# francescofugazzi/3dgsconverter

Measured on AMD Instinct MI355X. Metric: Msplats/sec SOR k=16, higher is better.
Workload: dtype f32 select / f64 finalize

## Files before the change

3dgsconverter_amd/csrc/knn_mfma.h:

```cpp
#pragma once

#include <hip/hip_runtime.h>

namespace gsx {

__device__ __forceinline__ unsigned shift_in_lt(unsigned m, float qx, float qy, float qz, float px, float py,
                                                float pz, float neg_tau)
{
    const float dx = qx - px, dy = qy - py, dz = qz - pz;
    const float t = __builtin_fmaf(dz, dz, __builtin_fmaf(dy, dy, __builtin_fmaf(dx, dx, neg_tau)));
    return __builtin_amdgcn_alignbit(m, __float_as_uint(t), 31);
}

typedef __bf16 bf16x8 __attribute__((ext_vector_type(8)));
typedef float f32x16 __attribute__((ext_vector_type(16)));
typedef unsigned u32x4 __attribute__((ext_vector_type(4)));
constexpr float MF_SLACK = 1e-3f;

__device__ __forceinline__ unsigned cvt_pk_bf16(float lo, float hi)
{
    unsigned r;
    asm("v_cvt_pk_bf16_f32 %0, %1, %2" : "=v"(r) : "v"(lo), "v"(hi));
    return r;
}
__device__ __forceinline__ float bf_lo(unsigned w) { return __uint_as_float(w << 16); }
__device__ __forceinline__ float bf_hi(unsigned w) { return __uint_as_float(w & 0xffff0000u); }

__host__ __device__ constexpr int mf_cand_of_row(int r) { return (r & 3) | (((r >> 3) & 3) << 2) | (((r >> 2) & 1) << 4); }

__device__ __forceinline__ bf16x8 mf_candidate_operand(float ux, float uy, float uz, bool upper)
{
    const unsigned l0 = cvt_pk_bf16(ux, ux);
    const float lx = ux - bf_lo(l0);
    const unsigned l1 = cvt_pk_bf16(lx, uy);
    const float ly = uy - bf_hi(l1);
    const unsigned l2 = cvt_pk_bf16(uy, ly);
    const unsigned l3 = cvt_pk_bf16(uz, uz);
    const float lz = uz - bf_lo(l3);
    const float n = __builtin_fmaf(uz, uz, __builtin_fmaf(uy, uy, ux * ux));
    const unsigned u0 = cvt_pk_bf16(lz, n);
    const float r1 = n - bf_hi(u0);
    const unsigned t = cvt_pk_bf16(r1, r1);
    const float r2 = r1 - bf_lo(t);
    const unsigned u1 = cvt_pk_bf16(r1, r2);
    u32x4 w;
    w.x = upper ? u0 : l0;
    w.y = upper ? u1 : l1;
    w.z = upper ? 0x3f803f80u : l2;
    w.w = upper ? 0x00003f80u : l3;
    return __builtin_bit_cast(bf16x8, w);
}

__device__ __forceinline__ void mf_query_operands(float ux, float uy, float uz, float s, bf16x8 &out_a, bf16x8 &out_b)
{
    const unsigned hx = cvt_pk_bf16(ux, uy);
    const unsigned hz = cvt_pk_bf16(uz, uz);
    const float hxf = bf_lo(hx), hyf = bf_hi(hx), hzf = bf_lo(hz);
    const float lx = ux - hxf, ly = uy - hyf, lz = uz - hzf;
    u32x4 lo, up;
    lo.x = cvt_pk_bf16(-2.0f * hxf, -2.0f * lx);
    lo.y = cvt_pk_bf16(-2.0f * hxf, -2.0f * hyf);
    lo.z = cvt_pk_bf16(-2.0f * ly, -2.0f * hyf);
    lo.w = cvt_pk_bf16(-2.0f * hzf, -2.0f * lz);
    const unsigned t1 = cvt_pk_bf16(s, s);
    const float r1 = s - bf_lo(t1);
    const unsigned t2 = cvt_pk_bf16(r1, r1);
    const float r2 = r1 - bf_lo(t2);
    up.x = cvt_pk_bf16(-2.0f * hzf, 1.0f);
    up.y = 0x3f803f80u;
    up.z = cvt_pk_bf16(s, r1);
    up.w = cvt_pk_bf16(r2, 0.0f);
    u32x4 a, b;
#pragma unroll
    for (int i = 0; i < 4; ++i) {
        auto r = __builtin_amdgcn_permlane32_swap(lo[i], up[i], false, false);
        a[i] = r[0];
        b[i] = r[1];
    }
    out_a = __builtin_bit_cast(bf16x8, a);
    out_b = __builtin_bit_cast(bf16x8, b);
}

__device__ __forceinline__ unsigned mf_sign_bits(const f32x16 &acc)
{
    unsigned m = 0;
#pragma unroll
    for (int r = 0; r < 16; ++r) m = __builtin_amdgcn_alignbit(m, __float_as_uint(acc[r]), 31);
    return m;
}

__device__ __forceinline__ void wave_sync()
{
    __builtin_amdgcn_fence(__ATOMIC_ACQ_REL, "wavefront");
    __builtin_amdgcn_wave_barrier();
}

}
```

3dgsconverter_amd/csrc/sor_grid.hip:

```cpp
#include <algorithm>
#include <chrono>
#include <cmath>
#include <cstdlib>
#include <type_traits>
#include <unordered_map>
#include <vector>

#include "gsx_common.h"
#include "knn_common.h"
#include "knn_mfma.h"
#include "sor_grid_params.h"

namespace gsx {


constexpr int MAX_DIM = 1024;
constexpr int MAX_BUCKETS = 4096;
constexpr int MAX_BUCKET_CELLS = 4096;
#ifndef GSX_BUCKET_POINTS
#define GSX_BUCKET_POINTS 4096
#endif
constexpr int BUCKET_POINTS = GSX_BUCKET_POINTS;
#ifndef GSX_BIN_TILE
#define GSX_BIN_TILE 8192
// ... 556 lines not shown
}

#ifndef GSX_SORT_THREADS
#define GSX_SORT_THREADS 512
#endif
#ifndef GSX_SORT_PPT
#define GSX_SORT_PPT 16
#endif
constexpr int SORT_THREADS = GSX_SORT_THREADS;
constexpr int SORT_PPT = GSX_SORT_PPT;
constexpr unsigned SORT_CAP = SORT_THREADS * SORT_PPT;

__device__ __forceinline__ int quarter_coord(float v, float o, float inv_h, int dim)
{
    int c = (int)((v - o) * (4.0f * inv_h));
    return min(max(c, 0), 4 * dim - 1);
}

template <bool FINE>
__global__ __launch_bounds__(SORT_THREADS) void bucket_sort_kernel(const GridParams *__restrict__ gp,
                                                          const unsigned *__restrict__ bk_start,
                                                          const float4 *__restrict__ in, float4 *__restrict__ out,
                                                          unsigned *__restrict__ cell_start, unsigned big_limit,
                                                          unsigned *__restrict__ fine_start)
{
    constexpr int SUB = FINE ? 4 : 1;
    __shared__ unsigned cnt[SUB * MAX_BUCKET_CELLS];
    __shared__ unsigned wsum[SORT_THREADS / 64];
    const GridParams g = *gp;
    const int b = blockIdx.x;
    if (g.bad_input || b >= g.bk_count) return;
    const int ncell = g.bk_cells;
    const int cells = SUB * ncell;
    const unsigned s0 = bk_start[b], s1 = bk_start[b + 1];
    if (b == g.bk_count - 1 && threadIdx.x == 0) {
        cell_start[(size_t)g.bk_count * ncell] = s1;
        if (FINE) fine_start[(size_t)g.bk_count * cells] = s1;
    }
    if (s1 - s0 > big_limit) return;
    const int by = b % g.bk_ny, bz = b / g.bk_ny;
    for (int i = threadIdx.x; i < cells; i += SORT_THREADS) cnt[i] = 0;
    __syncthreads();
    auto local_cell = [&](const float4 p) {
        const int cx = FINE ? quarter_coord(p.x, g.ox, g.inv_h, g.nx) : cell_coord(p.x, g.ox, g.inv_h, g.nx);
        const int cy = cell_coord(p.y, g.oy, g.inv_h, g.ny);
        const int cz = cell_coord(p.z, g.oz, g.inv_h, g.nz);
        return ((cz - bz * g.bk_g) * g.bk_g + (cy - by * g.bk_g)) * (SUB * g.nx) + cx;
    };
    const bool fits = s1 - s0 <= SORT_CAP;
    float4 p[SORT_PPT];
    int cell[SORT_PPT];
    unsigned rk[SORT_PPT];
    if (fits) {
#pragma unroll
        for (int u = 0; u < SORT_PPT; ++u) p[u] = in[min(s0 + u * SORT_THREADS + threadIdx.x, s1 - 1)];
#pragma unroll
        for (int u = 0; u < SORT_PPT; ++u) {
            cell[u] = local_cell(p[u]);
            rk[u] = s0 + u * SORT_THREADS + threadIdx.x < s1 ? atomicAdd(&cnt[cell[u]], 1u) : 0u;
        }
    } else {
        for (unsigned i = s0 + threadIdx.x; i < s1; i += SORT_THREADS) atomicAdd(&cnt[local_cell(in[i])], 1u);
    }
    __syncthreads();
    const int seg = (cells + SORT_THREADS - 1) / SORT_THREADS;
    const int c0 = min(cells, (int)threadIdx.x * seg), c1 = min(cells, c0 + seg);
    unsigned sum = 0;
    for (int c = c0; c < c1; ++c) sum += cnt[c];
    unsigned inc = sum;
#pragma unroll
    for (int off = 1; off < 64; off <<= 1) {
        unsigned o = __shfl_up(inc, off);
        if ((int)(threadIdx.x & 63) >= off) inc += o;
    }
    const int wv = threadIdx.x >> 6;
    if ((threadIdx.x & 63) == 63) wsum[wv] = inc;
    __syncthreads();
    unsigned run = inc - sum;
    for (int i = 0; i < wv; ++i) run += wsum[i];
    __syncthreads();
    for (int c = c0; c < c1; ++c) {
        const unsigned v = cnt[c];
        cnt[c] = run;
        run += v;
    }
    __syncthreads();
    unsigned *cs = cell_start + (size_t)b * ncell;
    for (int i = threadIdx.x; i < ncell; i += SORT_THREADS) cs[i] = s0 + cnt[SUB * i];
    if (FINE) {
        unsigned *fs = fine_start + (size_t)b * cells;
        for (int i = threadIdx.x; i < cells; i += SORT_THREADS) fs[i] = s0 + cnt[i];
    }
    if (fits) {
#pragma unroll
        for (int u = 0; u < SORT_PPT; ++u)
            if (s0 + u * SORT_THREADS + threadIdx.x < s1) out[s0 + cnt[cell[u]] + rk[u]] = p[u];
    } else {
        __syncthreads();
        for (unsigned i = s0 + threadIdx.x; i < s1; i += SORT_THREADS) {
            const float4 q = in[i];
            out[s0 + atomicAdd(&cnt[local_cell(q)], 1u)] = q;
        }
    }
}

constexpr unsigned BIG_BUCKET = 32768;
constexpr int BIG_CHUNK = 8192;

__device__ __forceinline__ int bucket_containing(const unsigned *bk_start, int nb, unsigned pos)
{
    int lo = 0, hi = nb;
    while (hi - lo > 1) {
        const int mid = (lo + hi) >> 1;
        if (bk_start[mid] <= pos) lo = mid; else hi = mid;
    }
    return lo;
}

template <bool SCATTER>
__global__ __launch_bounds__(256) void big_bucket_kernel(const GridParams *__restrict__ gp, const unsigned *__restrict__ bk_start,
                                                         int n, const float4 *__restrict__ in, float4 *__restrict__ out,
                                                         unsigned *cell_start ,
                                                         unsigned *cursor )
{
    __shared__ unsigned cnt[MAX_BUCKET_CELLS];
    __shared__ unsigned base[SCATTER ? MAX_BUCKET_CELLS : 1];
    const GridParams g = *gp;
    if (g.bad_input) return;
    const unsigned lo = (unsigned)blockIdx.x * BIG_CHUNK;
    if (lo >= (unsigned)n) return;
    const unsigned hi = min((unsigned)n, lo + BIG_CHUNK);
    const int cells = g.bk_cells;
    for (int b = bucket_containing(bk_start, g.bk_count, lo); b < g.bk_count; ++b) {
        const unsigned s0 = bk_start[b], s1 = bk_start[b + 1];
        if (s0 >= hi) break;
        if (s1 - s0 <= BIG_BUCKET) continue;
        const unsigned p0 = max(lo, s0), p1 = min(hi, s1);
        const int by = b % g.bk_ny, bz = b / g.bk_ny;
        auto local_cell = [&](const float4 p) {
            const int cx = cell_coord(p.x, g.ox, g.inv_h, g.nx);
            const int cy = cell_coord(p.y, g.oy, g.inv_h, g.ny);
            const int cz = cell_coord(p.z, g.oz, g.inv_h, g.nz);
            return ((cz - bz * g.bk_g) * g.bk_g + (cy - by * g.bk_g)) * g.nx + cx;
        };
        for (int i = threadIdx.x; i < cells; i += 256) cnt[i] = 0;
        __syncthreads();
        for (unsigned i = p0 + threadIdx.x; i < p1; i += 256) atomicAdd(&cnt[local_cell(in[i])], 1u);
        __syncthreads();
        unsigned *gc = (SCATTER ? cursor : cell_start) + (size_t)b * cells;
        for (int i = threadIdx.x; i < cells; i += 256) {
            const unsigned c = cnt[i];
            if (c) {
                const unsigned r = atomicAdd(&gc[i], c);
                if (SCATTER) base[i] = r;
            }
            if (SCATTER) cnt[i] = 0;
        }
        __syncthreads();
        if (SCATTER) {
            for (unsigned i = p0 + threadIdx.x; i < p1; i += 256) {
                const float4 p = in[i];
                const int c = local_cell(p);
                out[base[c] + atomicAdd(&cnt[c], 1u)] = p;
            }
            __syncthreads();
        }
    }
}

__global__ __launch_bounds__(256) void big_bucket_scan_kernel(const GridParams *__restrict__ gp,
                                                              const unsigned *__restrict__ bk_start,
                                                              unsigned *cell_start, unsigned *cursor)
{
    __shared__ unsigned wsum[4];
    const GridParams g = *gp;
    const int b = blockIdx.x;
    if (g.bad_input || b >= g.bk_count) return;
    const unsigned s0 = bk_start[b], s1 = bk_start[b + 1];
    if (s1 - s0 <= BIG_BUCKET) return;
    const int cells = g.bk_cells;
    unsigned *cs = cell_start + (size_t)b * cells, *cu = cursor + (size_t)b * cells;
    const int seg = (cells + 255) / 256;
    const int c0 = min(cells, (int)threadIdx.x * seg), c1 = min(cells, c0 + seg);
    unsigned sum = 0;
    for (int c = c0; c < c1; ++c) sum += cs[c];
    unsigned tot;
    unsigned run = s0 + block_exclusive_scan_256(sum, &tot, wsum);
    for (int c = c0; c < c1; ++c) {
        const unsigned v = cs[c];
        cs[c] = run;
        cu[c] = run;
        run += v;
    }
}

constexpr int PLAN_MAXQ = 64;
constexpr int PLAN_MAXRUN = 10;
constexpr int PLAN_WAVES = 4;

template <bool WRITE>
__global__ __launch_bounds__(64 * PLAN_WAVES) void brick_plan_kernel(GridParams *__restrict__ gp, const unsigned *__restrict__ fine_start,
                                                                     unsigned *__restrict__ bundle_cnt, unsigned *__restrict__ bundle_off,
                                                                     uint2 *__restrict__ list)
{
    __shared__ unsigned s_sum[PLAN_WAVES][MAX_DIM + 1];
    __shared__ unsigned short s_nxt[PLAN_WAVES][MAX_DIM];
    __shared__ unsigned wsum[4];
    __shared__ unsigned s_last;
    const GridParams g = *gp;
    if (g.bad_input || !g.plan) return;
    const int lane = threadIdx.x & 63, wv = threadIdx.x >> 6;
    unsigned *S = s_sum[wv];
    unsigned short *nxt = s_nxt[wv];
    const int nq4 = 4 * g.nx, nbund = g.nby * g.nbz;
    const unsigned cap = (unsigned)g.plan_cap;
    constexpr int QPL = MAX_DIM / 64 + 1;
    for (int bundle = (int)blockIdx.x * PLAN_WAVES + wv; bundle < nbund; bundle += (int)gridDim.x * PLAN_WAVES) {
        const int bz = bundle / g.nby, by = bundle - bz * g.nby;
        int rb[4];
#pragma unroll
        for (int r = 0; r < 4; ++r) {
            const int yy = 2 * by + (r & 1), zz = 2 * bz + (r >> 1);
            rb[r] = yy < g.ny && zz < g.nz ? 4 * row_base(g, yy, zz) : -1;
        }
        unsigned v[QPL][4];
#pragma unroll
        for (int u = 0; u < QPL; ++u) {
            const int q = lane + 64 * u;
#pragma unroll
            for (int r = 0; r < 4; ++r) v[u][r] = (q <= nq4 && rb[r] >= 0) ? fine_start[rb[r] + q] : 0u;
        }
#pragma unroll
        for (int u = 0; u < QPL; ++u) {
            const int q = lane + 64 * u;
            if (q <= nq4) S[q] = v[u][0] + v[u][1] + v[u][2] + v[u][3];
        }
        wave_sync();
        for (int s = lane; s < nq4; s += 64) {
            const unsigned s0 = S[s];
            int e = s + 1;
#pragma unroll
            for (int j = 2; j <= PLAN_MAXRUN; ++j) e += (s + j <= nq4 && S[min(s + j, nq4)] - s0 <= (unsigned)PLAN_MAXQ) ? 1 : 0;
            nxt[s] = (unsigned short)e;
        }
        wave_sync();
        if (lane == 0) {
            const unsigned base = WRITE ? bundle_off[bundle] : 0u;
            unsigned n = 0;
            for (int s = 0; s < nq4; ++n) {
                const int e = nxt[s];
                if (WRITE && base + n < cap) list[base + n] = make_uint2((unsigned)bundle, (unsigned)s | ((unsigned)(e - 1) << 16));
                s = e;
            }
            if (!WRITE) __hip_atomic_store(&bundle_cnt[bundle], n, __ATOMIC_RELAXED, __HIP_MEMORY_SCOPE_AGENT);
        }
        wave_sync();
    }
    if (WRITE) return;
    __builtin_amdgcn_s_waitcnt(0);
    __syncthreads();
    if (threadIdx.x == 0) s_last = atomicAdd(&gp->ticket_plan, 1u) == gridDim.x - 1 ? 1u : 0u;
    __syncthreads();
    if (!s_last) return;
    constexpr int HOLD = 16;
    const int seg = (nbund + 255) / 256;
    const int c0 = min(nbund, (int)threadIdx.x * seg), c1 = min(nbund, c0 + seg);
    const bool held = seg <= HOLD;
    unsigned hv[HOLD];
    unsigned sum = 0;
    for (int c = c0; c < c1; c += HOLD) {
#pragma unroll
        for (int u = 0; u < HOLD; ++u) hv[u] = c + u < c1 ? __hip_atomic_load(&bundle_cnt[c + u], __ATOMIC_RELAXED, __HIP_MEMORY_SCOPE_AGENT) : 0u;
#pragma unroll
        for (int u = 0; u < HOLD; ++u) sum += hv[u];
    }
    unsigned tot;
    unsigned run = block_exclusive_scan_256(sum, &tot, wsum);
    for (int c = c0; c < c1; c += HOLD) {
        unsigned w[HOLD];
#pragma unroll
        for (int u = 0; u < HOLD; ++u)
            w[u] = held ? hv[u] : (c + u < c1 ? __hip_atomic_load(&bundle_cnt[c + u], __ATOMIC_RELAXED, __HIP_MEMORY_SCOPE_AGENT) : 0u);
#pragma unroll
        for (int u = 0; u < HOLD; ++u) {
            if (c + u < c1) bundle_off[c + u] = run;
            run += w[u];
        }
    }
    if (threadIdx.x == 0) {
        gp->ticket_plan = 0;
        if (tot > cap) {
            gp->plan = 0;
        } else {
            gp->nbricks = (int)tot;
            gp->part_lo = 0;
            gp->part_hi = (int)tot;
        }
    }
}

#ifndef GSX_NET_WAVES17
#define GSX_NET_WAVES17 5
#endif
#ifndef GSX_BRICK_UNROLL3
#define GSX_BRICK_UNROLL3 0
#endif
#ifndef GSX_NET_WAVES33
#define GSX_NET_WAVES33 4
#endif
#ifndef GSX_NET_HB
#define GSX_NET_HB 4
#endif
#ifndef GSX_NET_WAVES25
#define GSX_NET_WAVES25 4
#endif
#ifndef GSX_NET_WAVES49
#define GSX_NET_WAVES49 3
#endif
constexpr int NET_WAVES9 = 5, NET_WAVES17 = GSX_NET_WAVES17, NET_WAVES25 = GSX_NET_WAVES25, NET_WAVES33 = GSX_NET_WAVES33,
              NET_WAVES49 = GSX_NET_WAVES49;
constexpr int NET_HB = GSX_NET_HB;
constexpr int brick_min_waves(int kcap, bool mf, bool net)
{
    (void)mf;
    if (net) return kcap <= 9 ? NET_WAVES9 : (kcap <= 17 ? NET_WAVES17 : (kcap <= 25 ? NET_WAVES25 : (kcap <= 33 ? NET_WAVES33 : (kcap <= 49 ? NET_WAVES49 : 2))));
    return kcap <= 17 ? 5 : (kcap <= 26 ? 4 : (kcap <= 33 ? 3 : 2));
}

template <int KCAP, bool EXTRA, bool MF, bool NET, bool PLAN = false>
__global__ __launch_bounds__(BRICK_THREADS, brick_min_waves(KCAP, MF, NET)) void knn_brick_kernel(
    GridParams *__restrict__ gp, const float4 *__restrict__ refs, const unsigned *__restrict__ rstart,
    const float4 *__restrict__ qpts, const unsigned *__restrict__ qstart, int k, int q_begin,
    float *__restrict__ mean_out, unsigned *__restrict__ faillist, uint2 *__restrict__ extra,
    unsigned *__restrict__ deferred, double *__restrict__ kth_out, const uint2 *__restrict__ plist)
{
    constexpr int WCAP = KCAP > 33 ? GSX_WCAP_BIG : (KCAP > 17 ? GSX_WCAP_MID : gsx::WCAP);
    __shared__ unsigned s_mask[BRICK_THREADS / 64][WCAP][64];
    __shared__ unsigned s_wbase[BRICK_THREADS / 64][WCAP];
    __shared__ uint2 s_wseg[MF ? BRICK_THREADS / 64 : 1][MF ? WCAP : 1];

    if (EXTRA && gp->extra_count == 0) return;
    const int lane = lane_id();
    const int wv = uniform((int)(threadIdx.x >> 6));
    unsigned(*mask)[64] = s_mask[wv];
    unsigned *wbase = s_wbase[wv];
    uint2 *wseg = s_wseg[MF ? wv : 0];

    const int nx = gp->nx, ny = gp->ny, nz = gp->nz;
    const int nbx = gp->nbx, nby = gp->nby;
    const int bdx = gp->bdx, bdy = gp->bdy, bdz = gp->bdz;
    const int cry = bdy + 2;
    const int ncrows = cry * (bdz + 2);
    const int nqrows = bdy * bdz;
    const double r1sq = gp->r1sq;
    const double hp = gp->hprime;
    const float tau1 = gp->tau1;
    const float g_ox = gp->ox, g_oy = gp->oy, g_oz = gp->oz, g_inv_h = gp->inv_h;
    const int bk_g = gp->bk_g, bk_ny = gp->bk_ny, bk_cells = gp->bk_cells;
    auto row_base_g = [&](int cy, int cz) {
        const int by_ = cy / bk_g, bz_ = cz / bk_g;
        return (bz_ * bk_ny + by_) * bk_cells + ((cz - bz_ * bk_g) * bk_g + (cy - by_ * bk_g)) * nx;
    };
#ifdef GSX_ABLATE
    const int dbg = gp->debug_skip;
#else
    constexpr int dbg = 0;
#endif
    const int kk = k + 1;
    const int kq = NET ? k : kk;

    WorkQueue wq;
    const int part_lo = gp->part_lo;
    const int nq4 = 4 * nx;
    const bool planned = PLAN && gp->plan != 0;
    const int dw = EXTRA ? 0 : gp->defer_words;
    wq_init(wq, EXTRA ? gp->extra_ctr : gp->brick_ctr, EXTRA ? (int)gp->extra_count : gp->part_hi - part_lo,
            BRICK_THREADS / 64);
    for (;;) {
        const int item = uniform(wq_next(wq));
        if (item < 0) break;
        int b = item + part_lo, qb = 0;
        if (EXTRA) {
            const uint2 it = extra[item];
            b = uniform((int)it.x);
            qb = uniform((int)it.y);
        }
        int bx, by, bz;
        int qf = 0, ql = 0;
        if constexpr (PLAN) {
            int bundle;
            if (planned) {
                const uint2 e = plist[b];
                bundle = uniform((int)e.x);
                qf = uniform((int)(e.y & 0xffffu));
                ql = uniform((int)(e.y >> 16));
            } else {
                bundle = b / nbx;
                qf = 8 * (b - bundle * nbx);
                ql = min(qf + 7, nq4 - 1);
            }
            bz = bundle / nby;
            by = bundle - bz * nby;
            bx = 0;
        } else {
            bz = b / (nbx * nby);
            const int brem = b - bz * nbx * nby;
            by = brem / nbx;
            bx = brem - by * nbx;
        }

        int v_start = 0, v_len = 0;
        {
            const int ln = pinned_here(lane);
            const bool isq = ln >= 16;
            const int r = isq ? ln - 16 : ln;
            const int r_mod_bdy = bdy == 2 ? (r & 1) : 0, r_div_bdy = bdy == 2 ? (r >> 1) : r;
            const int r_div_cry = cry == 4 ? (r >> 2) : (r * 11) >> 5;
            const int r_mod_cry = r - r_div_cry * cry;
            const int yy = isq ? by * bdy + r_mod_bdy : by * bdy - 1 + r_mod_cry;
            const int zz = isq ? bz * bdz + r_div_bdy : bz * bdz - 1 + r_div_cry;
            const int xa = PLAN ? (isq ? qf : max(qf - 4, 0)) : (isq ? bx * bdx : max(bx * bdx - 1, 0));
            const int xb = PLAN ? (isq ? ql : min(ql + 4, nq4 - 1))
                                : (isq ? min(bx * bdx + bdx - 1, nx - 1) : min(bx * bdx + bdx, nx - 1));
            const bool valid = (isq ? (lane < 20 && r < nqrows) : r < ncrows) && yy >= 0 && yy < ny && zz >= 0 && zz < nz;
            if (valid) {
                const unsigned *st = isq ? qstart : rstart;
                const int row = PLAN ? 4 * row_base_g(yy, zz) : row_base_g(yy, zz);
                unsigned s = st[row + xa], e = st[row + xb + 1];
                v_start = (int)s;
                v_len = (int)(e - s);
            }
        }
        if (dbg & 16) continue;
        int qoff[5];
        qoff[0] = 0;
#pragma unroll
        for (int r = 0; r < 4; ++r) qoff[r + 1] = qoff[r] + __builtin_amdgcn_readlane(v_len, 16 + r);
        const int nq = qoff[4];
        if (!EXTRA) {
            if (dw > 0 && nq > 0) {
                int ncand = 0;
#pragma unroll
                for (int r = 0; r < 16; ++r) ncand += __builtin_amdgcn_readlane(v_len, r);
                const int words = (ncand + 31) >> 5, batches = (nq + 63) >> 6;
                if (words > dw || (long long)words * batches > 2LL * dw) {
                    if (lane == 0) deferred[atomicAdd(&gp->deferred_count, 1u)] = (unsigned)b;
                    continue;
                }
            }
        }
        constexpr int LOCAL_MAX = 3;
        const int LOCAL_BATCHES = nq > 64 * LOCAL_MAX ? 1 : LOCAL_MAX;
        if (!EXTRA && nq > 64 * LOCAL_BATCHES) {
            const int nextra = (nq - 1) / 64 + 1 - LOCAL_BATCHES;
            unsigned slot = 0;
            if (lane == 0) slot = atomicAdd(&gp->extra_count, (unsigned)nextra);
            slot = (unsigned)uniform((int)slot);
            for (int e = lane; e < nextra; e += 64)
                extra[slot + e] = make_uint2((unsigned)b, (unsigned)(64 * (e + LOCAL_BATCHES)));
        }
        const int qb_end = EXTRA ? min(nq, qb + 64) : min(nq, 64 * LOCAL_BATCHES);

        for (; qb < qb_end; qb += 64) {
            const int f = qb + lane;
            const bool live = f < nq;
            int qidx = 0;
#pragma unroll
            for (int r = 0; r < 4; ++r) {
                int s = __builtin_amdgcn_readlane(v_start, 16 + r);
                if (f >= qoff[r] && f < qoff[r + 1]) qidx = s + (f - qoff[r]);
            }
            const float4 qp = qpts[live ? qidx : 0];
            const float qx = qp.x, qy = qp.y, qz = qp.z;
            const bool is_query = live && !(__float_as_uint(qp.w) >> 31);
            if (!__any(is_query)) continue;
            float tau = is_query ? tau1 : -1.0f;
            double racc_sq = r1sq;
            {
                const int ulo[3] = {bx * bdx - 1, by * bdy - 1, bz * bdz - 1};
                const int uhi[3] = {bx * bdx + bdx, by * bdy + bdy, bz * bdz + bdz};
                const int dim[3] = {nx, ny, nz};
                const bool boundary = (PLAN ? qf - 4 <= 0 || ql + 4 >= nq4 - 1 : ulo[0] <= 0 || uhi[0] >= nx - 1) || ulo[1] <= 0 ||
                                      ulo[2] <= 0 || uhi[1] >= ny - 1 || uhi[2] >= nz - 1;
                if (boundary && qb == 0) {
                    const float hf = pinned_here((float)hp);
                    const int pbx = pinned_here_s(bx), pby = pinned_here_s(by), pbz = pinned_here_s(bz);
                    const int ulo[3] = {pbx * bdx - 1, pby * bdy - 1, pbz * bdz - 1};
                    const int uhi[3] = {pbx * bdx + bdx, pby * bdy + bdy, pbz * bdz + bdz};
                    const float rel[3] = {qx - g_ox, qy - g_oy, qz - g_oz};
                    const float r1 = hf * (1.0f - 1e-3f);
                    float rsafe = 3.0e38f, frac = 1.0f;
#pragma unroll
                    for (int a = 0; a < 3; ++a) {
                        if (PLAN && a == 0) {
                            const int pqf = pinned_here_s(qf), pql = pinned_here_s(ql);
                            if (pqf - 4 > 0) rsafe = fminf(rsafe, rel[0] - (float)(pqf - 4) * 0.25f * hf - 2e-3f * hf);
                            if (pql + 4 < nq4 - 1) rsafe = fminf(rsafe, (float)(pql + 5) * 0.25f * hf - rel[0] - 2e-3f * hf);
                        } else {
                        if (ulo[a] > 0) rsafe = fminf(rsafe, rel[a] - (float)ulo[a] * hf - 2e-3f * hf);
                        if (uhi[a] < dim[a] - 1) rsafe = fminf(rsafe, (float)(uhi[a] + 1) * hf - rel[a] - 2e-3f * hf);
                        }
                        const float tl = fminf(fmaxf(rel[a], 0.0f), r1);
                        const float th = fminf(fmaxf((float)dim[a] * hf - rel[a], 0.0f), r1);
                        frac *= (tl + th) / (2.0f * r1);
                    }
                    float rq = r1 * cbrtf(1.0f / fmaxf(frac, 0.125f));
                    rq = fminf(rq, rsafe);
                    if (rq > r1 && is_query) {
                        racc_sq = (double)rq * (double)rq;
                        tau = bound_from(racc_sq);
                    }
                }
            }

            int rs_start = v_start, rs_len = v_len;
            if (qb > 0) {
                int lo[3], hi[3];
                const int c3[3] = {cell_coord(qx, g_ox, g_inv_h, nx), cell_coord(qy, g_oy, g_inv_h, ny),
                                   cell_coord(qz, g_oz, g_inv_h, nz)};
#pragma unroll
                for (int a = 0; a < 3; ++a) {
                    lo[a] = is_query ? c3[a] : 0x7fffffff;
                    hi[a] = is_query ? c3[a] : -1;
#pragma unroll
                    for (int off = 32; off > 0; off >>= 1) {
                        lo[a] = min(lo[a], __shfl_xor(lo[a], off));
                        hi[a] = max(hi[a], __shfl_xor(hi[a], off));
                    }
                    lo[a] = uniform(lo[a]);
                    hi[a] = uniform(hi[a]);
                }
                rs_start = 0;
                rs_len = 0;
                if (lane < ncrows) {
                    const int ln = pinned_here(lane);
                    const int l_div_cry = cry == 4 ? (ln >> 2) : (ln * 11) >> 5;
                    const int yy = by * bdy - 1 + (ln - l_div_cry * cry);
                    const int zz = bz * bdz - 1 + l_div_cry;
                    const int xa = PLAN ? max(max(qf - 4, 0), 4 * (lo[0] - 1)) : max(max(bx * bdx - 1, 0), lo[0] - 1);
                    const int xb = PLAN ? min(min(ql + 4, nq4 - 1), 4 * (hi[0] + 1) + 3) : min(min(bx * bdx + bdx, nx - 1), hi[0] + 1);
                    const bool need = yy >= max(lo[1] - 1, 0) && yy <= min(hi[1] + 1, ny - 1) &&
                                      zz >= max(lo[2] - 1, 0) && zz <= min(hi[2] + 1, nz - 1) && xa <= xb;
                    if (need) {
                        const int row = PLAN ? 4 * row_base_g(yy, zz) : row_base_g(yy, zz);
                        const unsigned s0 = rstart[row + xa], e0 = rstart[row + xb + 1];
                        rs_start = (int)s0;
                        rs_len = (int)(e0 - s0);
                    }
                }
            }
            typename std::conditional<NET, TopNet<NET ? KCAP - 1 : 8>, TopList<KCAP>>::type lst;
            bool lst_empty = true;

            int widx = 0;
            unsigned nzw = 0;

            auto drain = [&]() __attribute__((always_inline)) {
                const double qxd = (double)qx, qyd = (double)qy, qzd = (double)qz;
                wave_sync();
                if (dbg & 32) nzw = 0;
                unsigned m = 0;
                int base = 0, c1 = 32, base2 = 0;
                if constexpr (NET) {
                    using Net = TopNet<NET ? KCAP - 1 : 8>;
                    constexpr int BS = Net::BS, HB = NET_HB < BS ? NET_HB : BS;
                    const unsigned self_w = __float_as_uint(qp.w);
                    for (;;) {
                        double blk[BS];
#pragma unroll
                        for (int h0 = 0; h0 < BS; h0 += HB) {
                            float4 pt[HB];
                            bool ok[HB];
#pragma unroll
                            for (int j = 0; j < HB; ++j) {
                                if (m == 0 && nzw != 0) {
                                    const int w = __builtin_ctz(nzw);
                                    nzw &= nzw - 1;
                                    m = mask[w][lane];
                                    base = (int)wbase[w];
                                    if constexpr (MF) {
                                        const uint2 sg = wseg[w];
                                        c1 = (int)sg.x;
                                        base2 = (int)sg.y;
                                    }
                                }
                                ok[j] = m != 0;
                                const int i = ok[j] ? __builtin_clz(m) : 0;
                                m &= ~(0x80000000u >> i);
                                const int idx = (MF && i >= c1 ? base2 : base) + i;
                                if constexpr (MF && NET) pt[j] = *(const float4 *)((const char *)refs + ((unsigned)idx << 4));
                                else pt[j] = refs[idx];
                            }
#pragma unroll
                            for (int j = 0; j < HB; ++j) {
                                double d = dist2_f64(qxd, qyd, qzd, pt[j].x, pt[j].y, pt[j].z);
                                blk[h0 + j] = (ok[j] && __float_as_uint(pt[j].w) != self_w) ? d : __builtin_inf();
                            }
                        }
                        if (uniform((int)lst_empty)) lst.assign_block(blk); else lst.merge_block(blk);
                        lst_empty = false;
                        if (!__any(m != 0 || nzw != 0)) break;
                    }
                } else {
                bool have_cur = false;
                float4 pc = make_float4(0.f, 0.f, 0.f, 0.f);
                for (;;) {
                    if (m == 0 && nzw != 0) {
                        const int w = __builtin_ctz(nzw);
                        nzw &= nzw - 1;
                        m = mask[w][lane];
                        base = (int)wbase[w];
                        if constexpr (MF) {
                            const uint2 sg = wseg[w];
                            c1 = (int)sg.x;
                            base2 = (int)sg.y;
                        }
                    }
                    const bool have_next = m != 0;
                    float4 pn = pc;
                    if (have_next) {
                        const int i = __builtin_clz(m);
                        m &= ~(0x80000000u >> i);
                        pn = refs[(MF && i >= c1 ? base2 : base) + i];
                    }
                    if (have_cur && !(dbg & 1)) lst.insert(dist2_f64(qxd, qyd, qzd, pc.x, pc.y, pc.z));
                    if (!__any(have_next)) break;
                    pc = pn;
                    have_cur = have_next;
                }
                }
                tau = fminf(tau, bound_from(lst.kth(kq)));
                widx = 0;
                nzw = 0;
                wave_sync();
            };

            bool mf_done = false;
            if constexpr (MF) {
                int nwords = 0;
                {
                    int fill = 0, segs = 0;
                    for (int r = 0; r < ncrows; ++r) {
                        int len = __builtin_amdgcn_readlane(rs_len, r & 15);
                        while (len > 0) {
                            if (fill == 32 || segs == 2) {
                                ++nwords;
                                fill = 0;
                                segs = 0;
                            }
                            const int take = min(len, 32 - fill);
                            fill += take;
                            len -= take;
                            ++segs;
                        }
                    }
                    nwords += fill > 0;
                }
                if (nwords <= WCAP && !(dbg & 2)) {
                mf_done = true;
                const float hf = pinned_here((float)hp);
                const float ccx = PLAN ? g_ox + ((float)(qf + ql + 1) * 0.125f) * hf : g_ox + ((float)(bx * bdx) + 0.5f * (float)bdx) * hf;
                const float ccy = g_oy + ((float)(by * bdy) + 0.5f * (float)bdy) * hf;
                const float ccz = g_oz + ((float)(bz * bdz) + 0.5f * (float)bdz) * hf;
                const float uqx = (qx - ccx) * g_inv_h, uqy = (qy - ccy) * g_inv_h, uqz = (qz - ccz) * g_inv_h;
                const float nq2 = __builtin_fmaf(uqz, uqz, __builtin_fmaf(uqy, uqy, uqx * uqx));
                const bool upper = lane >= 32;
                const float s_q = tau >= 0.0f ? nq2 - ((tau * g_inv_h) * g_inv_h * (1.0f + 1e-6f) + MF_SLACK) : 1.0e30f;
                bf16x8 opa, opb;
                mf_query_operands(uqx, uqy, uqz, s_q, opa, opb);
                const int nrows = ncrows;
                struct Word { int b1, c1, b2, c2, r, off; };
                auto next_word = [&](int r, int off) __attribute__((always_inline)) {
                    Word o{0, 0, 0, 0, r, off};
                    int len = r < nrows ? __builtin_amdgcn_readlane(rs_len, r & 15) : 0;
                    while (r < nrows && off >= len) {
                        ++r;
                        off = 0;
                        len = r < nrows ? __builtin_amdgcn_readlane(rs_len, r & 15) : 0;
                    }
                    if (r < nrows) {
                        o.b1 = __builtin_amdgcn_readlane(rs_start, r & 15) + off;
                        o.c1 = min(32, len - off);
                        off += o.c1;
                        if (o.c1 < 32) {
                            do {
                                ++r;
                                off = 0;
                                len = r < nrows ? __builtin_amdgcn_readlane(rs_len, r & 15) : 0;
                            } while (r < nrows && len == 0);
                            if (r < nrows) {
                                o.b2 = __builtin_amdgcn_readlane(rs_start, r & 15);
                                o.c2 = min(32 - o.c1, len);
                                off = o.c2;
                            }
                        }
                    }
                    o.r = r;
                    o.off = off;
                    return o;
                };
                const int my_cand = mf_cand_of_row(lane & 31);
                auto fetch = [&](const Word &w) __attribute__((always_inline)) {
                    const int c = w.c1 + w.c2;
                    if (c == 0) return make_float4(0.f, 0.f, 0.f, 0.f);
                    const int t = min(my_cand, c - 1);
                    const int idx = t < w.c1 ? w.b1 + t : w.b2 + (t - w.c1);
                    if constexpr (NET) return *(const float4 *)((const char *)refs + ((unsigned)idx << 4));
                    else return refs[idx];
                };
                auto process = [&](const Word &w_cur, const float4 &p_cur) __attribute__((always_inline)) {
                    const bf16x8 cand = mf_candidate_operand((p_cur.x - ccx) * g_inv_h, (p_cur.y - ccy) * g_inv_h,
                                                             (p_cur.z - ccz) * g_inv_h, upper);
                    const f32x16 zero = {0.f, 0.f, 0.f, 0.f, 0.f, 0.f, 0.f, 0.f, 0.f, 0.f, 0.f, 0.f, 0.f, 0.f, 0.f, 0.f};
                    const unsigned ma = mf_sign_bits(__builtin_amdgcn_mfma_f32_32x32x16_bf16(cand, opa, zero, 0, 0, 0));
                    const unsigned mb = mf_sign_bits(__builtin_amdgcn_mfma_f32_32x32x16_bf16(cand, opb, zero, 0, 0, 0));
                    auto sw = __builtin_amdgcn_permlane32_swap(ma, mb, false, false);
                    const unsigned m = ((sw[0] << 16) | (sw[1] & 0xffffu)) & (0xffffffffu << (32 - (w_cur.c1 + w_cur.c2)));
                    if (dbg & 64) atomicAdd(&gp->exhaustive_count, (unsigned)__builtin_popcount(m));
                    mask[widx][lane] = m;
                    if (lane == 0) {
                        wbase[widx] = (unsigned)w_cur.b1;
                        wseg[widx] = make_uint2((unsigned)w_cur.c1, (unsigned)(w_cur.b2 - w_cur.c1));
                    }
                    nzw |= (m != 0 ? 1u : 0u) << widx;
                    ++widx;
                };
#if GSX_BRICK_UNROLL3
                Word w0 = next_word(0, 0);
                Word w1 = next_word(w0.r, w0.off), w2;
                float4 p0 = fetch(w0), p1 = fetch(w1), p2;
                for (;;) {
                    if (!(w0.c1 > 0)) break;
                    w2 = next_word(w1.r, w1.off);
                    p2 = fetch(w2);
                    process(w0, p0);
                    if (!(w1.c1 > 0)) break;
                    w0 = next_word(w2.r, w2.off);
                    p0 = fetch(w0);
                    process(w1, p1);
                    if (!(w2.c1 > 0)) break;
                    w1 = next_word(w0.r, w0.off);
                    p1 = fetch(w1);
                    process(w2, p2);
                }
#else
                Word w_cur = next_word(0, 0);
                Word w_n1 = next_word(w_cur.r, w_cur.off);
                float4 p_cur = fetch(w_cur), p_n1 = fetch(w_n1);
                while (w_cur.c1 > 0) {
                    const Word w_n2 = next_word(w_n1.r, w_n1.off);
                    const float4 p_n2 = fetch(w_n2);
                    process(w_cur, p_cur);
                    w_cur = w_n1;
                    p_cur = p_n1;
                    w_n1 = w_n2;
                    p_n1 = p_n2;
                }
#endif
                lst.init();
                }
            }
            if (!mf_done) {
            lst.init();
            for (int r = 0; r < ((dbg & 2) ? 0 : ncrows); ++r) {
                const int gs = __builtin_amdgcn_readlane(rs_start, r);
                const int len = __builtin_amdgcn_readlane(rs_len, r);
                for (int w0 = 0; w0 < len; w0 += 32) {
                    if (widx == WCAP) drain();
                    const int c = min(32, len - w0);
                    const float4 *__restrict__ p = refs + gs + w0;
                    const float neg_tau = -tau;
                    unsigned m = 0;
                    int i = 0;
                    struct Quad { float4 v[4]; };
                    const Quad *__restrict__ pq = reinterpret_cast<const Quad *>(p);
                    for (; i + 8 <= c; i += 8) {
                        const Quad a = pq[i / 4], b = pq[i / 4 + 1];
#pragma unroll
                        for (int u = 0; u < 4; ++u) m = shift_in_lt(m, qx, qy, qz, a.v[u].x, a.v[u].y, a.v[u].z, neg_tau);
#pragma unroll
                        for (int u = 0; u < 4; ++u) m = shift_in_lt(m, qx, qy, qz, b.v[u].x, b.v[u].y, b.v[u].z, neg_tau);
                    }
                    for (; i < c; ++i) {
                        float4 P = p[i];
                        m = shift_in_lt(m, qx, qy, qz, P.x, P.y, P.z, neg_tau);
                    }
                    m <<= (32 - c);
                    if (dbg & 64) atomicAdd(&gp->exhaustive_count, (unsigned)__builtin_popcount(m));
                    mask[widx][lane] = m;
                    if (lane == 0) {
                        wbase[widx] = (unsigned)(gs + w0);
                        if constexpr (MF) wseg[widx] = make_uint2(32u, 0u);
                    }
                    nzw |= (m != 0 ? 1u : 0u) << widx;
                    ++widx;
                }
            }
            }
            drain();

            if (is_query) {
                const double kth_d2 = lst.kth(kq);
                if (dbg & 8) {
                    if (kth_d2 == 12345.0) mean_out[0] = 1.0f;
                } else if (dbg & 4) {
                    mean_out[(int)__float_as_uint(qp.w) - q_begin] = (float)kth_d2;
                } else if (kth_d2 <= racc_sq) {
                    kth_emit(gp, kth_out, (int)__float_as_uint(qp.w) - q_begin, kth_d2, qx, qy, qz);
                    if constexpr (NET) mean_out[(int)__float_as_uint(qp.w) - q_begin] = mean_from_net(lst, k);
                    else mean_out[(int)__float_as_uint(qp.w) - q_begin] = mean_from_list<KCAP>(lst, k);
                } else {
                    unsigned slot = atomicAdd(&gp->fail_count, 1u);
                    faillist[slot] = (unsigned)qidx;
                }
            }
        }
    }
}

__device__ __forceinline__ double wave_min_f64(double v)
{
#pragma unroll
    for (int off = 32; off > 0; off >>= 1) {
        double o = __shfl_xor(v, off);
        v = o < v ? o : v;
    }
    return v;
}

constexpr int RING_ROWS = 320;

template <int KCAP>
__global__ __launch_bounds__(BRICK_THREADS) void knn_ring_kernel(
    GridParams *__restrict__ gp, const float4 *__restrict__ refs, const unsigned *__restrict__ rstart,
    const float4 *__restrict__ qpts, const unsigned *__restrict__ faillist, int k, int q_begin,
    float *__restrict__ mean_out, double *__restrict__ kth_out, unsigned *__restrict__ heavylist, int out_count, int after_fast)
{
    __shared__ double s_out[BRICK_THREADS / 64][KCAP];
    __shared__ int s_rs[BRICK_THREADS / 64][RING_ROWS];
    __shared__ int s_ro[BRICK_THREADS / 64][RING_ROWS + 1];
    const int lane = lane_id();
    const int wv = uniform((int)(threadIdx.x >> 6));
    double *out = s_out[wv];
    int *rs = s_rs[wv], *ro = s_ro[wv];
    const GridParams g = *gp;
    if (g.bad_input) {
        for (int i = blockIdx.x * blockDim.x + threadIdx.x; i < out_count; i += gridDim.x * blockDim.x)
            mean_out[i] = __builtin_nanf("");
        return;
    }
    const int nfail = (int)(after_fast ? g.ring2_count : g.fail_count);
    if (nfail == 0) return;
    const int kk = k + 1;

    WorkQueue wq;
    wq_init(wq, gp->ring_ctr, nfail, BRICK_THREADS / 64);
    for (;;) {
        const int t = uniform(wq_next(wq));
        if (t < 0) break;
        const unsigned fq = faillist[t];
        const float4 qp = qpts[fq];
        const double qxd = (double)qp.x, qyd = (double)qp.y, qzd = (double)qp.z;
        const int cx = cell_coord(qp.x, g.ox, g.inv_h, g.nx);
        const int cy = cell_coord(qp.y, g.oy, g.inv_h, g.ny);
        const int cz = cell_coord(qp.z, g.oz, g.inv_h, g.nz);

        for (int H = 2;; H *= 2) {
            double a[KCAP];
#pragma unroll
            for (int i = 0; i < KCAP; ++i) a[i] = __builtin_inf();
            auto consider = [&](const float4 p) __attribute__((always_inline)) {
                double d = dist2_f64(qxd, qyd, qzd, p.x, p.y, p.z);
                if (d < a[KCAP - 1]) {
#pragma unroll
                    for (int i = 0; i < KCAP; ++i) {
                        double lo, hi;
                        asm("v_min_f64 %0, %1, %2" : "=v"(lo) : "v"(a[i]), "v"(d));
                        asm("v_max_f64 %0, %1, %2" : "=v"(hi) : "v"(a[i]), "v"(d));
                        a[i] = lo;
                        d = hi;
                    }
                }
            };
            const int x0 = max(cx - H, 0), x1 = min(cx + H, g.nx - 1);
            const int y0 = max(cy - H, 0), y1 = min(cy + H, g.ny - 1);
            const int z0 = max(cz - H, 0), z1 = min(cz + H, g.nz - 1);
            const int nyr = y1 - y0 + 1;
            const int nrows = nyr * (z1 - z0 + 1);
            if (nrows <= RING_ROWS) {
                int carry = 0;
                for (int r0 = 0; r0 < nrows; r0 += 64) {
                    const int r = r0 + lane;
                    int s = 0, len = 0;
                    if (r < nrows) {
                        const int zz = z0 + r / nyr, yy = y0 + r % nyr;
                        const int row = row_base(g, yy, zz);
                        s = (int)rstart[row + x0];
                        len = (int)rstart[row + x1 + 1] - s;
                    }
                    int inc = len;
#pragma unroll
                    for (int off = 1; off < 64; off <<= 1) {
                        int o = __shfl_up(inc, off);
                        if (lane >= off) inc += o;
                    }
                    if (r < nrows) {
                        rs[r] = s;
                        ro[r] = carry + inc - len;
                    }
                    carry += __shfl(inc, 63);
                }
                const int total = carry;
                if (g.heavy_limit > 0 && total > g.heavy_limit) {
                    if (lane == 0) heavylist[atomicAdd(&gp->heavy_count, 1u)] = fq;
                    break;
                }
                if (lane == 0) ro[nrows] = total;
                wave_sync();
                int row = 0;
                for (int f0 = lane; f0 < total; f0 += 256) {
                    float4 p[4];
                    bool ok[4];
#pragma unroll
                    for (int u = 0; u < 4; ++u) {
                        const int f = f0 + 64 * u;
                        ok[u] = f < total;
                        if (ok[u]) {
                            while (f >= ro[row + 1]) ++row;
                            p[u] = refs[rs[row] + (f - ro[row])];
                        }
                    }
#pragma unroll
                    for (int u = 0; u < 4; ++u)
                        if (ok[u]) consider(p[u]);
                }
            } else {
                if (g.heavy_limit > 0) {
                    int total = 0;
                    for (int r = lane; r < nrows; r += 64) {
                        const int row = row_base(g, y0 + r % nyr, z0 + r / nyr);
                        total += (int)(rstart[row + x1 + 1] - rstart[row + x0]);
                    }
#pragma unroll
                    for (int off = 32; off > 0; off >>= 1) total += __shfl_xor(total, off);
                    if (uniform(total) > g.heavy_limit) {
                        if (lane == 0) heavylist[atomicAdd(&gp->heavy_count, 1u)] = fq;
                        break;
                    }
                }
                for (int zz = z0; zz <= z1; ++zz)
                    for (int yy = y0; yy <= y1; ++yy) {
                        const int row = row_base(g, yy, zz);
                        const int s = (int)rstart[row + x0], e = (int)rstart[row + x1 + 1];
                        for (int j = s + lane; j < e; j += 64) consider(refs[j]);
                    }
            }
            for (int r = 0; r < kk; ++r) {
                const double mn = wave_min_f64(a[0]);
                const unsigned long long eq = __ballot(a[0] == mn);
                const int win = (int)__builtin_ctzll(eq);
                if (lane == 0) out[r] = mn;
                if (lane == win) {
#pragma unroll
                    for (int i = 0; i + 1 < KCAP; ++i) a[i] = a[i + 1];
                    a[KCAP - 1] = __builtin_inf();
                }
            }
            wave_sync();
            const bool covers = x0 == 0 && y0 == 0 && z0 == 0 && x1 == g.nx - 1 && y1 == g.ny - 1 && z1 == g.nz - 1;
            const double rH = (double)H * g.hprime * (1.0 - 1e-3);
            const double kth = out[kk - 1];
            if (covers || kth <= rH * rH) {
                for (int i = lane; i < kk; i += 64) out[i] = __dsqrt_rn(out[i]);
                wave_sync();
                if (lane == 0) {
                    if (covers && !(kth <= rH * rH)) atomicAdd(&gp->exhaustive_count, 1u);
                    double sum = pairwise_sum_le128([&](int i) { return out[1 + i]; }, k);
                    mean_out[(int)__float_as_uint(qp.w) - q_begin] = __double2float_rn(__ddiv_rn(sum, (double)k));
                    kth_emit(gp, kth_out, (int)__float_as_uint(qp.w) - q_begin, kth, qp.x, qp.y, qp.z);
                }
                wave_sync();
                break;
            }
            wave_sync();
        }
    }
}

constexpr int ANYK_MAX = 2048;

template <int DEPTH, class F>
__device__ double pairwise_sum_np(F at, int lo, int n)
{
    if constexpr (DEPTH == 0) {
        return pairwise_sum_le128([&](int i) { return at(lo + i); }, n);
    } else {
        if (n <= 128) return pairwise_sum_le128([&](int i) { return at(lo + i); }, n);
        int n2 = n / 2;
        n2 -= n2 % 8;
        return __dadd_rn(pairwise_sum_np<DEPTH - 1>(at, lo, n2), pairwise_sum_np<DEPTH - 1>(at, lo + n2, n - n2));
    }
}

__global__ __launch_bounds__(BRICK_THREADS) void knn_anyk_kernel(GridParams *__restrict__ gp, const float4 *__restrict__ refs,
                                                                 const unsigned *__restrict__ rstart, const float4 *__restrict__ qpts,
                                                                 int nq, int k, int q_begin, float *__restrict__ mean_out,
                                                                 double *__restrict__ kth_out)
{
    __shared__ unsigned s_hist[BRICK_THREADS / 64][256];
    __shared__ double s_sel[BRICK_THREADS / 64][ANYK_MAX];
    __shared__ unsigned s_cnt[BRICK_THREADS / 64];
    const int lane = lane_id();
    const int wv = uniform((int)(threadIdx.x >> 6));
    unsigned *hist = s_hist[wv];
    double *sel = s_sel[wv];
    const GridParams g = *gp;
    const int kk = k + 1;
    const int nwaves = gridDim.x * (BRICK_THREADS / 64);
    if (g.bad_input) {
        for (int i = blockIdx.x * blockDim.x + threadIdx.x; i < nq; i += gridDim.x * blockDim.x) mean_out[i] = __builtin_nanf("");
        return;
    }
    for (int t = blockIdx.x * (BRICK_THREADS / 64) + wv; t < nq; t += nwaves) {
        const float4 qp = qpts[t];
        if (__float_as_uint(qp.w) >> 31) continue;
        const double qxd = (double)qp.x, qyd = (double)qp.y, qzd = (double)qp.z;
        const int cx = cell_coord(qp.x, g.ox, g.inv_h, g.nx);
        const int cy = cell_coord(qp.y, g.oy, g.inv_h, g.ny);
        const int cz = cell_coord(qp.z, g.oz, g.inv_h, g.nz);
        for (int H = 1;; ++H) {
            const int x0 = max(cx - H, 0), x1 = min(cx + H, g.nx - 1);
            const int y0 = max(cy - H, 0), y1 = min(cy + H, g.ny - 1);
            const int z0 = max(cz - H, 0), z1 = min(cz + H, g.nz - 1);
            const bool covers = x0 == 0 && y0 == 0 && z0 == 0 && x1 == g.nx - 1 && y1 == g.ny - 1 && z1 == g.nz - 1;
            auto for_each = [&](auto f) __attribute__((always_inline)) {
                for (int zz = z0; zz <= z1; ++zz)
                    for (int yy = y0; yy <= y1; ++yy) {
                        const int row = row_base(g, yy, zz);
                        const int sb = (int)rstart[row + x0], se = (int)rstart[row + x1 + 1];
                        for (int j = sb + lane; j < se; j += 64) {
                            const float4 p = refs[j];
                            f((unsigned long long)__double_as_longlong(dist2_f64(qxd, qyd, qzd, p.x, p.y, p.z)));
                        }
                    }
            };
            unsigned long long prefix = 0ull, pmask = 0ull;
            int remaining = kk;
            bool enough = true;
            for (int pass = 0; pass < 8 && enough; ++pass) {
                const int shift = 56 - 8 * pass;
                for (int i = lane; i < 256; i += 64) hist[i] = 0u;
                wave_sync();
                for_each([&](unsigned long long b) {
                    if ((b & pmask) == prefix) atomicAdd(&hist[(unsigned)(b >> shift) & 255u], 1u);
                });
                wave_sync();
                const unsigned c0 = hist[4 * lane], c1 = hist[4 * lane + 1], c2 = hist[4 * lane + 2], c3 = hist[4 * lane + 3];
                unsigned inc = c0 + c1 + c2 + c3;
                const unsigned mine = inc;
#pragma unroll
                for (int off = 1; off < 64; off <<= 1) {
                    const unsigned o = __shfl_up(inc, off);
                    if (lane >= off) inc += o;
                }
                const unsigned total = __shfl(inc, 63);
                if (pass == 0 && (int)total < kk) {
// ... 1283 lines not shown
```

Baseline: 5542.

## Pair candidate words per wave half and fast-path word count via DPP

The MFMA candidate loop now processes two 32-candidate words per iteration. The lower half-wave fetches points for word A and the upper half for word B, and one candidate-operand build plus a permlane32 swap produces both MFMA operands. This removes the redundant per-lane point fetch and conversion that had each half computing only its own part. The word count is first estimated with a DPP prefix sum over row lengths, and the exact serial packing loop runs only when that estimate exceeds capacity. The 3-way unroll variant is removed and lst.init is hoisted.

Result: faster. 5910 (median of 6 runs) (+6.6%).

```diff
diff --git a/3dgsconverter_amd/csrc/knn_mfma.h b/3dgsconverter_amd/csrc/knn_mfma.h
--- a/3dgsconverter_amd/csrc/knn_mfma.h
+++ b/3dgsconverter_amd/csrc/knn_mfma.h
@@ -51,6 +51,35 @@
     return __builtin_bit_cast(bf16x8, w);
 }
 
+__device__ __forceinline__ void mf_candidate_operands_pair(float ux, float uy, float uz, bf16x8 &word_a, bf16x8 &word_b)
+{
+    u32x4 lo, up;
+    lo.x = cvt_pk_bf16(ux, ux);
+    const float lx = ux - bf_lo(lo.x);
+    lo.y = cvt_pk_bf16(lx, uy);
+    const float ly = uy - bf_hi(lo.y);
+    lo.z = cvt_pk_bf16(uy, ly);
+    lo.w = cvt_pk_bf16(uz, uz);
+    const float lz = uz - bf_lo(lo.w);
+    const float n = __builtin_fmaf(uz, uz, __builtin_fmaf(uy, uy, ux * ux));
+    up.x = cvt_pk_bf16(lz, n);
+    const float r1 = n - bf_hi(up.x);
+    const unsigned t = cvt_pk_bf16(r1, r1);
+    const float r2 = r1 - bf_lo(t);
+    up.y = cvt_pk_bf16(r1, r2);
+    up.z = 0x3f803f80u;
+    up.w = 0x00003f80u;
+    u32x4 a, b;
+#pragma unroll
+    for (int i = 0; i < 4; ++i) {
+        auto r = __builtin_amdgcn_permlane32_swap(lo[i], up[i], false, false);
+        a[i] = r[0];
+        b[i] = r[1];
+    }
+    word_a = __builtin_bit_cast(bf16x8, a);
+    word_b = __builtin_bit_cast(bf16x8, b);
+}
+
 __device__ __forceinline__ void mf_query_operands(float ux, float uy, float uz, float s, bf16x8 &out_a, bf16x8 &out_b)
 {
     const unsigned hx = cvt_pk_bf16(ux, uy);
diff --git a/3dgsconverter_amd/csrc/sor_grid.hip b/3dgsconverter_amd/csrc/sor_grid.hip
--- a/3dgsconverter_amd/csrc/sor_grid.hip
+++ b/3dgsconverter_amd/csrc/sor_grid.hip
@@ -882,9 +882,6 @@
 #ifndef GSX_NET_WAVES17
 #define GSX_NET_WAVES17 5
 #endif
-#ifndef GSX_BRICK_UNROLL3
-#define GSX_BRICK_UNROLL3 0
-#endif
 #ifndef GSX_NET_WAVES33
 #define GSX_NET_WAVES33 4
 #endif
@@ -1217,8 +1214,14 @@
 
             bool mf_done = false;
             if constexpr (MF) {
-                int nwords = 0;
-                {
+                int nwords = lane < 16 ? (rs_len + 31) >> 5 : 0;
+                nwords += __builtin_amdgcn_update_dpp(0, nwords, 0x111, 0xf, 0xf, true);
+                nwords += __builtin_amdgcn_update_dpp(0, nwords, 0x112, 0xf, 0xf, true);
+                nwords += __builtin_amdgcn_update_dpp(0, nwords, 0x114, 0xf, 0xf, true);
+                nwords += __builtin_amdgcn_update_dpp(0, nwords, 0x118, 0xf, 0xf, true);
+                nwords = __builtin_amdgcn_readlane(nwords, 15);
+                if (nwords > WCAP) {
+                    nwords = 0;
                     int fill = 0, segs = 0;
                     for (int r = 0; r < ncrows; ++r) {
                         int len = __builtin_amdgcn_readlane(rs_len, r & 15);
@@ -1280,68 +1283,55 @@
                     return o;
                 };
                 const int my_cand = mf_cand_of_row(lane & 31);
-                auto fetch = [&](const Word &w) __attribute__((always_inline)) {
-                    const int c = w.c1 + w.c2;
-                    if (c == 0) return make_float4(0.f, 0.f, 0.f, 0.f);
+                auto fetch = [&](const Word &wa, const Word &wb) __attribute__((always_inline)) {
+                    if (wa.c1 == 0) return make_float4(0.f, 0.f, 0.f, 0.f);
+                    const Word &wu = wb.c1 > 0 ? wb : wa;
+                    const int b1 = upper ? wu.b1 : wa.b1, c1 = upper ? wu.c1 : wa.c1;
+                    const int b2 = upper ? wu.b2 : wa.b2, c = upper ? wu.c1 + wu.c2 : wa.c1 + wa.c2;
                     const int t = min(my_cand, c - 1);
-                    const int idx = t < w.c1 ? w.b1 + t : w.b2 + (t - w.c1);
+                    const int idx = t < c1 ? b1 + t : b2 + (t - c1);
                     if constexpr (NET) return *(const float4 *)((const char *)refs + ((unsigned)idx << 4));
                     else return refs[idx];
                 };
-                auto process = [&](const Word &w_cur, const float4 &p_cur) __attribute__((always_inline)) {
-                    const bf16x8 cand = mf_candidate_operand((p_cur.x - ccx) * g_inv_h, (p_cur.y - ccy) * g_inv_h,
-                                                             (p_cur.z - ccz) * g_inv_h, upper);
+                auto park = [&](const Word &w, const bf16x8 &cand) __attribute__((always_inline)) {
                     const f32x16 zero = {0.f, 0.f, 0.f, 0.f, 0.f, 0.f, 0.f, 0.f, 0.f, 0.f, 0.f, 0.f, 0.f, 0.f, 0.f, 0.f};
                     const unsigned ma = mf_sign_bits(__builtin_amdgcn_mfma_f32_32x32x16_bf16(cand, opa, zero, 0, 0, 0));
                     const unsigned mb = mf_sign_bits(__builtin_amdgcn_mfma_f32_32x32x16_bf16(cand, opb, zero, 0, 0, 0));
                     auto sw = __builtin_amdgcn_permlane32_swap(ma, mb, false, false);
-                    const unsigned m = ((sw[0] << 16) | (sw[1] & 0xffffu)) & (0xffffffffu << (32 - (w_cur.c1 + w_cur.c2)));
+                    const unsigned m = ((sw[0] << 16) | (sw[1] & 0xffffu)) & (0xffffffffu << (32 - (w.c1 + w.c2)));
                     if (dbg & 64) atomicAdd(&gp->exhaustive_count, (unsigned)__builtin_popcount(m));
                     mask[widx][lane] = m;
                     if (lane == 0) {
-                        wbase[widx] = (unsigned)w_cur.b1;
-                        wseg[widx] = make_uint2((unsigned)w_cur.c1, (unsigned)(w_cur.b2 - w_cur.c1));
+                        wbase[widx] = (unsigned)w.b1;
+                        wseg[widx] = make_uint2((unsigned)w.c1, (unsigned)(w.b2 - w.c1));
                     }
                     nzw |= (m != 0 ? 1u : 0u) << widx;
                     ++widx;
                 };
-#if GSX_BRICK_UNROLL3
-                Word w0 = next_word(0, 0);
-                Word w1 = next_word(w0.r, w0.off), w2;
-                float4 p0 = fetch(w0), p1 = fetch(w1), p2;
-                for (;;) {
-                    if (!(w0.c1 > 0)) break;
-                    w2 = next_word(w1.r, w1.off);
-                    p2 = fetch(w2);
-                    process(w0, p0);
-                    if (!(w1.c1 > 0)) break;
-                    w0 = next_word(w2.r, w2.off);
-                    p0 = fetch(w0);
-                    process(w1, p1);
-                    if (!(w2.c1 > 0)) break;
-                    w1 = next_word(w0.r, w0.off);
-                    p1 = fetch(w1);
-                    process(w2, p2);
-                }
-#else
-                Word w_cur = next_word(0, 0);
-                Word w_n1 = next_word(w_cur.r, w_cur.off);
-                float4 p_cur = fetch(w_cur), p_n1 = fetch(w_n1);
-                while (w_cur.c1 > 0) {
-                    const Word w_n2 = next_word(w_n1.r, w_n1.off);
-                    const float4 p_n2 = fetch(w_n2);
-                    process(w_cur, p_cur);
-                    w_cur = w_n1;
+                auto process = [&](const Word &wa, const Word &wb, const float4 &p) __attribute__((always_inline)) {
+                    bf16x8 cand_a, cand_b;
+                    mf_candidate_operands_pair((p.x - ccx) * g_inv_h, (p.y - ccy) * g_inv_h, (p.z - ccz) * g_inv_h, cand_a, cand_b);
+                    park(wa, cand_a);
+                    if (wb.c1 > 0) park(wb, cand_b);
+                };
+                Word a_cur = next_word(0, 0), b_cur = next_word(a_cur.r, a_cur.off);
+                Word a_n1 = next_word(b_cur.r, b_cur.off), b_n1 = next_word(a_n1.r, a_n1.off);
+                float4 p_cur = fetch(a_cur, b_cur), p_n1 = fetch(a_n1, b_n1);
+                while (a_cur.c1 > 0) {
+                    const Word a_n2 = next_word(b_n1.r, b_n1.off), b_n2 = next_word(a_n2.r, a_n2.off);
+                    const float4 p_n2 = fetch(a_n2, b_n2);
+                    process(a_cur, b_cur, p_cur);
+                    a_cur = a_n1;
+                    b_cur = b_n1;
                     p_cur = p_n1;
-                    w_n1 = w_n2;
+                    a_n1 = a_n2;
+                    b_n1 = b_n2;
                     p_n1 = p_n2;
                 }
-#endif
-                lst.init();
-                }
-            }
+                }
+            }
+            lst.init();
             if (!mf_done) {
-            lst.init();
             for (int r = 0; r < ((dbg & 2) ? 0 : ncrows); ++r) {
                 const int gs = __builtin_amdgcn_readlane(rs_start, r);
                 const int len = __builtin_amdgcn_readlane(rs_len, r);
```
